# ltiao/bore

Measured on NVIDIA B200. Metric: mlp_value_and_input_grad_evals_per_sec, higher is better.
Workload: dtype f32 MLP / f64 L-BFGS-B

## Files before the change

### bore_b200/csrc/mlp_eval.cu

```cuda
#include <algorithm>

#include <stdlib.h>

#include "common.cuh"
#include "act.cuh"

namespace {

template <int UGB>
struct Map {
  static constexpr int UG = 1 << UGB;
  static constexpr int PG = 32 >> UGB;
  static constexpr int TP = 4 * PG;
  static constexpr int CH = 4 * UG;
  static constexpr int AST = TP + 4;
};

struct SmemPlan {
  int wf[BORE_MAX_LAYERS];
  int bias[BORE_MAX_LAYERS];
  int wl;
  int weights_total;
  int buf[BORE_MAX_LAYERS];
  int warp_total;
  int wl_len;
};

__host__ __device__ inline int rup(int a, int b) { return (a + b - 1) / b * b; }

__host__ __device__ inline void make_plan(const MlpDesc &d, bool grad, int CH, int AST, SmemPlan &p) {
  int off = 0;
  const int G = d.n_layers - 1;
  for (int l = 0; l < G; ++l) {
    int in = d.dims[l], out = d.dims[l + 1];
    p.wf[l] = off; off += (grad ? rup(in, CH) : rup(in, 4)) * (rup(out, CH) + 4);
    p.bias[l] = off; off += rup(out, CH);
  }
  p.wl_len = G > 0 ? rup(d.dims[G], CH) : rup(d.dims[0], CH / 4);
  p.wl = off; off += p.wl_len;
  p.weights_total = rup(off, 4);
  int w = 0;
  p.buf[0] = 0; w += AST * (G > 0 ? rup(d.dims[0], 4) : p.wl_len);
  for (int l = 1; l <= G; ++l) { p.buf[l] = w; w += AST * rup(d.dims[l], CH); }
  p.warp_total = w;
}

__device__ __forceinline__ uint64_t pk2(float lo, float hi) {
  uint64_t r;
  asm("mov.b64 %0, {%1, %2};" : "=l"(r) : "f"(lo), "f"(hi));
  return r;
}
__device__ __forceinline__ void fma2(uint64_t &c, uint64_t a, uint64_t b) {
  asm("fma.rn.f32x2 %0, %1, %2, %0;" : "+l"(c) : "l"(a), "l"(b));
}
__device__ __forceinline__ float2 upk2(uint64_t v) {
  float2 r;
  asm("mov.b64 {%0, %1}, %2;" : "=f"(r.x), "=f"(r.y) : "l"(v));
  return r;
}

template <int AST, bool F2>
__device__ __forceinline__ void tile_gemm(const float *__restrict__ A, const float *__restrict__ W,
                                          int K4, int ldw, float (&acc)[4][4]) {
  if (F2) {
    uint64_t c2[2][4];
#pragma unroll
    for (int u = 0; u < 4; ++u) { c2[0][u] = pk2(acc[0][u], acc[1][u]); c2[1][u] = pk2(acc[2][u], acc[3][u]); }
#pragma unroll 2
    for (int k = 0; k < K4; k += 4) {
      float4 a[4], w[4];
#pragma unroll
      for (int kk = 0; kk < 4; ++kk) {
        a[kk] = *reinterpret_cast<const float4 *>(A + (k + kk) * AST);
        w[kk] = *reinterpret_cast<const float4 *>(W + (k + kk) * ldw);
      }
#pragma unroll
      for (int kk = 0; kk < 4; ++kk) {
        const uint64_t a01 = pk2(a[kk].x, a[kk].y), a23 = pk2(a[kk].z, a[kk].w);
        const float wv[4] = {w[kk].x, w[kk].y, w[kk].z, w[kk].w};
#pragma unroll
        for (int u = 0; u < 4; ++u) {
          const uint64_t ww = pk2(wv[u], wv[u]);
          fma2(c2[0][u], a01, ww);
          fma2(c2[1][u], a23, ww);
        }
      }
    }
#pragma unroll
    for (int u = 0; u < 4; ++u) {
      const float2 lo = upk2(c2[0][u]), hi = upk2(c2[1][u]);
      acc[0][u] = lo.x; acc[1][u] = lo.y; acc[2][u] = hi.x; acc[3][u] = hi.y;
    }
    return;
  }
#pragma unroll 2
  for (int k = 0; k < K4; k += 4) {
    float4 a[4], w[4];
#pragma unroll
    for (int kk = 0; kk < 4; ++kk) {
      a[kk] = *reinterpret_cast<const float4 *>(A + (k + kk) * AST);
      w[kk] = *reinterpret_cast<const float4 *>(W + (k + kk) * ldw);
    }
#pragma unroll
    for (int kk = 0; kk < 4; ++kk) {
      const float av[4] = {a[kk].x, a[kk].y, a[kk].z, a[kk].w};
      const float wv[4] = {w[kk].x, w[kk].y, w[kk].z, w[kk].w};
#pragma unroll
      for (int i = 0; i < 4; ++i)
#pragma unroll
        for (int u = 0; u < 4; ++u) acc[i][u] = fmaf(av[i], wv[u], acc[i][u]);
    }
  }
}

template <int AST, int RS, bool F2>
__device__ __forceinline__ void tile_gemm_T(const float *__restrict__ A, const float *__restrict__ Wrow,
                                            int J4, int ldw, float (&acc)[4][4]) {
  if (F2) {
    uint64_t c2[2][4];
#pragma unroll
    for (int u = 0; u < 4; ++u) { c2[0][u] = pk2(acc[0][u], acc[1][u]); c2[1][u] = pk2(acc[2][u], acc[3][u]); }
#pragma unroll 2
    for (int j = 0; j < J4; j += 4) {
      float4 a[4], w[4];
#pragma unroll
      for (int jj = 0; jj < 4; ++jj) a[jj] = *reinterpret_cast<const float4 *>(A + (j + jj) * AST);
#pragma unroll
      for (int u = 0; u < 4; ++u) w[u] = *reinterpret_cast<const float4 *>(Wrow + u * RS * ldw + j);
#pragma unroll
      for (int jj = 0; jj < 4; ++jj) {
        const uint64_t a01 = pk2(a[jj].x, a[jj].y), a23 = pk2(a[jj].z, a[jj].w);
#pragma unroll
        for (int u = 0; u < 4; ++u) {
          const float wv = jj == 0 ? w[u].x : jj == 1 ? w[u].y : jj == 2 ? w[u].z : w[u].w;
          const uint64_t ww = pk2(wv, wv);
          fma2(c2[0][u], a01, ww);
          fma2(c2[1][u], a23, ww);
        }
      }
    }
#pragma unroll
    for (int u = 0; u < 4; ++u) {
      const float2 lo = upk2(c2[0][u]), hi = upk2(c2[1][u]);
      acc[0][u] = lo.x; acc[1][u] = lo.y; acc[2][u] = hi.x; acc[3][u] = hi.y;
    }
    return;
  }
#pragma unroll 2
  for (int j = 0; j < J4; j += 4) {
    float4 a[4], w[4];
#pragma unroll
    for (int jj = 0; jj < 4; ++jj) a[jj] = *reinterpret_cast<const float4 *>(A + (j + jj) * AST);
#pragma unroll
    for (int u = 0; u < 4; ++u) w[u] = *reinterpret_cast<const float4 *>(Wrow + u * RS * ldw + j);
#pragma unroll
    for (int jj = 0; jj < 4; ++jj) {
      const float av[4] = {a[jj].x, a[jj].y, a[jj].z, a[jj].w};
#pragma unroll
      for (int u = 0; u < 4; ++u) {
        const float wv = jj == 0 ? w[u].x : jj == 1 ? w[u].y : jj == 2 ? w[u].z : w[u].w;
#pragma unroll
        for (int i = 0; i < 4; ++i) acc[i][u] = fmaf(av[i], wv, acc[i][u]);
      }
    }
  }
}

__global__ void __launch_bounds__(256)
mlp_pack_kernel(const MlpDesc d, const SmemPlan P, int CH, int grad, const float *__restrict__ params_all,
                float *__restrict__ packed_all) {
  const float *params = params_all + (size_t)blockIdx.x * d.n_params;
  float *out = packed_all + (size_t)blockIdx.x * P.weights_total;
  const int G = d.n_layers - 1;
  const int tid = threadIdx.x, nthr = blockDim.x;
  for (int l = 0; l < G; ++l) {
    const int in = d.dims[l], outd = d.dims[l + 1];
    const int rows = grad ? rup(in, CH) : rup(in, 4), outP = rup(outd, CH), ld = outP + 4;
    const float *Wg = params + d.w_off[l];
    float *wf = out + P.wf[l];
    for (int e = tid; e < rows * ld; e += nthr) {
      const int k = e / ld, j = e - k * ld;
      wf[e] = (k < in && j < outd) ? Wg[k * outd + j] : 0.f;
    }
    float *bs = out + P.bias[l];
    for (int e = tid; e < outP; e += nthr) bs[e] = e < outd ? params[d.b_off[l] + e] : 0.f;
  }
  {
    const int in = d.dims[G];
    float *wl = out + P.wl;
    for (int e = tid; e < P.weights_total - P.wl; e += nthr)
      wl[e] = e < in ? params[d.w_off[G] + e] : 0.f;
  }
}

__device__ __forceinline__ uint32_t smem_addr(const void *p) { return (uint32_t)__cvta_generic_to_shared(p); }

template <bool GRAD, int UGB, bool F2, bool EXT>
__global__ void __launch_bounds__(512)
mlp_eval_kernel(const MlpDesc d, const SmemPlan P, const float *__restrict__ params,
                const float *__restrict__ packed, const float *__restrict__ X,
                int S, const int *__restrict__ n_dev, const int *__restrict__ list,
                float *__restrict__ f_out, float *__restrict__ g_out, int transform, float sign,
                int per_model, const int *__restrict__ flags) {
  extern __shared__ __align__(128) float smem[];
  __shared__ __align__(8) uint64_t s_bar;
  using M = Map<UGB>;
  constexpr int TP = M::TP, AST = M::AST, CH = M::CH, UG = M::UG;
  const int G = d.n_layers - 1;
  const int tid = threadIdx.x, nthr = blockDim.x;
  const bool multi = per_model > 0;
  int n, tile0, tile_step;
  long row_base = 0;
  int *llist = reinterpret_cast<int *>(smem + P.weights_total + (nthr >> 5) * P.warp_total);
  if (multi) {
    params += (size_t)blockIdx.x * d.n_params;
    packed += (size_t)blockIdx.x * P.weights_total;
    row_base = (long)blockIdx.x * per_model;
    if (flags) {
      __shared__ int s_cnt;
      if (tid == 0) s_cnt = 0;
      __syncthreads();
      for (int c0 = 0; c0 < per_model; c0 += nthr) {
        const int i = c0 + tid;
        const bool on = i < per_model && flags[row_base + i] != 0;
        const unsigned b = __ballot_sync(0xffffffffu, on);
        int wbase = 0;
        if ((tid & 31) == 0 && b) wbase = atomicAdd(&s_cnt, __popc(b));
        wbase = __shfl_sync(0xffffffffu, wbase, 0);
        if (on) llist[wbase + __popc(b & ((1u << (tid & 31)) - 1u))] = i;
      }
      __syncthreads();
      n = s_cnt;
      list = llist;
    } else {
      n = per_model;
      list = nullptr;
    }
    if (n == 0) return;
    tile0 = 0;
    tile_step = nthr >> 5;
  } else {
    n = n_dev ? min(*n_dev, S) : S;
    if (blockIdx.x * (nthr >> 5) * TP >= n) return;
    tile0 = blockIdx.x * (nthr >> 5);
    tile_step = gridDim.x * (nthr >> 5);
  }

  if (tid == 0) {
    const uint32_t bar = smem_addr(&s_bar);
    const uint32_t total = (uint32_t)P.weights_total * sizeof(float);
    asm volatile("mbarrier.init.shared::cta.b64 [%0], 1;" ::"r"(bar) : "memory");
    asm volatile("fence.mbarrier_init.release.cluster;" ::: "memory");
    asm volatile("mbarrier.arrive.expect_tx.shared::cta.b64 _, [%0], %1;" ::"r"(bar), "r"(total) : "memory");
    for (uint32_t off = 0; off < total; off += 65536u) {
      const uint32_t nb = total - off < 65536u ? total - off : 65536u;
      asm volatile("cp.async.bulk.shared::cluster.global.mbarrier::complete_tx::bytes [%0], [%1], %2, [%3];"
                   ::"r"(smem_addr(smem) + off), "l"(reinterpret_cast<const char *>(packed) + off), "r"(nb),
                     "r"(bar)
                   : "memory");
    }
  }
  __syncthreads();
  {
    const uint32_t bar = smem_addr(&s_bar);
    asm volatile(
        "{\n"
        ".reg .pred p;\n"
        "W_WAIT:\n"
        "mbarrier.try_wait.parity.shared::cta.b64 p, [%0], 0;\n"
        "@p bra W_DONE;\n"
        "bra W_WAIT;\n"
        "W_DONE:\n"
        "}\n" ::"r"(bar)
        : "memory");
  }
  const float b_last = params[d.b_off[G]];
  const int act_last = d.act[G];

  const int n_tiles = (n + TP - 1) / TP;
  const int warp = tid >> 5, lane = tid & 31, nwarps = nthr >> 5;
  const int ug = lane & (UG - 1), pg = lane >> UGB;
  float *strip = smem + P.weights_total + warp * P.warp_total;
  const int D = d.dims[0];
  const float *wl = smem + P.wl;

  for (int tile = tile0 + warp; tile < n_tiles; tile += tile_step) {
    const int p0 = tile * TP;
    {
      float *xb = strip + P.buf[0];
      const int rows0 = G > 0 ? rup(D, 4) : P.wl_len;
      for (int pl = 0; pl < TP; ++pl) {
        const int idx = p0 + pl;
        const bool ok = idx < n;
        const long row = ok ? row_base + (list ? list[idx] : idx) : 0;
        for (int k = lane; k < rows0; k += 32)
          xb[k * AST + pl] = (ok && k < D) ? X[row * D + k] : 0.f;
      }
    }
    __syncwarp();

    for (int l = 0; l < G; ++l) {
      const int in4 = rup(d.dims[l], 4), outP = rup(d.dims[l + 1], CH);
      const float *A = strip + P.buf[l] + pg * 4;
      float *H = strip + P.buf[l + 1];
      const float *W = smem + P.wf[l];
      const float *bs = smem + P.bias[l];
      const int a = d.act[l];
      for (int c = 0; c < outP; c += CH) {
        float acc[4][4] = {};
        tile_gemm<AST, F2>(A, W + c + ug * 4, in4, outP + 4, acc);
#pragma unroll
        for (int u = 0; u < 4; ++u) {
          const int unit = c + ug * 4 + u;
          const float b = bs[unit];
          float4 o;
          o.x = act_fwd<EXT>(a, acc[0][u] + b);
          o.y = act_fwd<EXT>(a, acc[1][u] + b);
          o.z = act_fwd<EXT>(a, acc[2][u] + b);
          o.w = act_fwd<EXT>(a, acc[3][u] + b);
          *reinterpret_cast<float4 *>(H + unit * AST + pg * 4) = o;
        }
      }
      __syncwarp();
    }

    float *HL = strip + P.buf[G];
    float up[4] = {0.f, 0.f, 0.f, 0.f};
    for (int k = ug; k < P.wl_len; k += UG) {
      const float4 hv = *reinterpret_cast<const float4 *>(HL + k * AST + pg * 4);
      const float w = wl[k];
      up[0] = fmaf(hv.x, w, up[0]);
      up[1] = fmaf(hv.y, w, up[1]);
      up[2] = fmaf(hv.z, w, up[2]);
      up[3] = fmaf(hv.w, w, up[3]);
    }
#pragma unroll
    for (int i = 0; i < 4; ++i) {
#pragma unroll
      for (int o = 1; o < UG; o <<= 1) up[i] += __shfl_xor_sync(0xffffffffu, up[i], o);
    }
    float dpre[4];
#pragma unroll
    for (int i = 0; i < 4; ++i) {
      const float u = act_fwd<EXT>(act_last, up[i] + b_last);
      float fval, dT;
      if (GRAD) {
        const float v = sign * u;
        if (transform == BORE_TRANSFORM_SIGMOID) {
          fval = 1.f / (1.f + expf(-v));
          dT = fval * (1.f - fval);
        } else if (transform == BORE_TRANSFORM_EXP) {
          fval = expf(v);
          dT = fval;
        } else {
          fval = v;
          dT = 1.f;
        }
        dpre[i] = dT * sign * act_bwd<EXT>(act_last, u);
      } else {
        fval = u;
      }
      const int idx = p0 + pg * 4 + i;
      if (ug == 0 && idx < n) f_out[row_base + (list ? list[idx] : idx)] = fval;
    }
    if (!GRAD) { __syncwarp(); continue; }

    if (G == 0) {
      for (int k = ug; k < D; k += UG) {
        const float w = wl[k];
#pragma unroll
        for (int i = 0; i < 4; ++i) {
          const int idx = p0 + pg * 4 + i;
          if (idx < n) g_out[(row_base + (list ? list[idx] : idx)) * D + k] = dpre[i] * w;
        }
      }
      __syncwarp();
      continue;
    }
    {
      const int a = d.act[G - 1];
      for (int k = ug; k < P.wl_len; k += UG) {
        float4 hv = *reinterpret_cast<const float4 *>(HL + k * AST + pg * 4);
        const float w = wl[k];
        hv.x = dpre[0] * w * act_bwd<EXT>(a, hv.x);
        hv.y = dpre[1] * w * act_bwd<EXT>(a, hv.y);
        hv.z = dpre[2] * w * act_bwd<EXT>(a, hv.z);
        hv.w = dpre[3] * w * act_bwd<EXT>(a, hv.w);
        *reinterpret_cast<float4 *>(HL + k * AST + pg * 4) = hv;
      }
    }
    __syncwarp();
    for (int l = G - 1; l >= 0; --l) {
      const int out4 = rup(d.dims[l + 1], 4), inP = rup(d.dims[l], CH), ldw = rup(d.dims[l + 1], CH) + 4;
      const float *A = strip + P.buf[l + 1] + pg * 4;
      const float *W = smem + P.wf[l];
      float *Hin = strip + P.buf[l];
      if (l > 0) {
        const int a = d.act[l - 1];
        for (int c = 0; c < inP; c += CH) {
          float acc[4][4] = {};
          tile_gemm_T<AST, UG, F2>(A, W + (c + ug) * ldw, out4, ldw, acc);
#pragma unroll
          for (int u = 0; u < 4; ++u) {
            float *hp = Hin + (c + ug + UG * u) * AST + pg * 4;
            float4 hv = *reinterpret_cast<const float4 *>(hp);
            hv.x = acc[0][u] * act_bwd<EXT>(a, hv.x);
            hv.y = acc[1][u] * act_bwd<EXT>(a, hv.y);
            hv.z = acc[2][u] * act_bwd<EXT>(a, hv.z);
            hv.w = acc[3][u] * act_bwd<EXT>(a, hv.w);
            *reinterpret_cast<float4 *>(hp) = hv;
          }
        }
        __syncwarp();
      } else {
        for (int c = 0; c < inP; c += CH) {
          float acc[4][4] = {};
          tile_gemm_T<AST, UG, F2>(A, W + (c + ug) * ldw, out4, ldw, acc);
#pragma unroll
          for (int u = 0; u < 4; ++u) {
            const int k = c + ug + UG * u;
            if (k < rup(D, 4))
              *reinterpret_cast<float4 *>(Hin + k * AST + pg * 4) =
                  make_float4(acc[0][u], acc[1][u], acc[2][u], acc[3][u]);
          }
        }
        __syncwarp();
        for (int pl = 0; pl < TP; ++pl) {
          const int idx = p0 + pl;
          if (idx >= n) break;
          const long row = row_base + (list ? list[idx] : idx);
          for (int k = lane; k < D; k += 32) g_out[row * D + k] = Hin[k * AST + pl];
        }
        __syncwarp();
      }
    }
  }
}

}

static int variant_index(bool grad, int UGB) { return (grad ? 2 : 0) + (UGB == 4 ? 1 : 0); }

template <bool GRAD, int UGB>
static int pack_variant(const bore_mlp *h, int model0, int n_models, cudaStream_t stream) {
  using M = Map<UGB>;
  SmemPlan P;
  make_plan(h->desc, GRAD, M::CH, M::AST, P);
  const int v = variant_index(GRAD, UGB);
  MlpPackCache *pc = h->pack;
  BORE_CHECK(pc != nullptr, "handle has no pack cache");
  const size_t need = (size_t)h->n_models * P.weights_total;
  if (pc->cap[v] < need) {
    if (pc->buf[v]) BORE_CUDA(cudaFree(pc->buf[v]));
    pc->buf[v] = nullptr; pc->cap[v] = 0;
    BORE_CUDA(cudaMalloc(&pc->buf[v], need * sizeof(float)));
    pc->cap[v] = need;
  }
  mlp_pack_kernel<<<n_models, 256, 0, stream>>>(h->desc, P, M::CH, GRAD ? 1 : 0,
                                                 h->params + (size_t)model0 * h->desc.n_params,
                                                 pc->buf[v] + (size_t)model0 * P.weights_total);
  BORE_CUDA(cudaGetLastError());
  return 0;
}

constexpr int EVAL_MAX_SMEM = 227 * 1024;
constexpr int EVAL_STATIC_SMEM = 256;

static size_t eval_smem_bytes(const SmemPlan &P, int warps, size_t list_bytes) {
  return (size_t)(P.weights_total + warps * P.warp_total) * sizeof(float) + list_bytes;
}

template <bool GRAD, int UGB>
static int launch_variant(const bore_mlp *h, const MlpDesc &d, int model0, const float *X,
                          int S, float *f, float *g, const int *list, const int *n_dev,
                          int transform, float sign, int n_models, int per_model, const int *flags,
                          int prepacked, cudaStream_t stream) {
  using M = Map<UGB>;
  SmemPlan P;
  make_plan(d, GRAD, M::CH, M::AST, P);
  const int max_smem = EVAL_MAX_SMEM;
  const bool multi = per_model > 0;
  const size_t list_bytes = (multi && flags) ? (size_t)per_model * sizeof(int) : 0;
  int warps = 16;
  if (multi) warps = std::min(16, std::max(1, (per_model + M::TP - 1) / M::TP));
  while (warps > 1 && eval_smem_bytes(P, warps, list_bytes) + EVAL_STATIC_SMEM > (size_t)max_smem) --warps;
  const size_t smem = eval_smem_bytes(P, warps, list_bytes);
  BORE_CHECK(smem + EVAL_STATIC_SMEM <= (size_t)max_smem, "mlp_eval: model needs %zu B of shared memory (> %d)",
             smem + EVAL_STATIC_SMEM, max_smem);
  if (!prepacked && pack_variant<GRAD, UGB>(h, model0, n_models, stream)) return -1;
  const float *params = h->params + (size_t)model0 * d.n_params;
  const float *packed = h->pack->buf[variant_index(GRAD, UGB)] + (size_t)model0 * P.weights_total;
  int grid;
  if (multi) {
    grid = n_models;
  } else {
    const int n_tiles = (S + M::TP - 1) / M::TP;
    int ctas_needed = (n_tiles + warps - 1) / warps;
    int per_sm = (int)((size_t)max_smem / (smem + 1024));
    if (per_sm < 1) per_sm = 1;
    if (per_sm * warps > 48) per_sm = 48 / warps > 0 ? 48 / warps : 1;
    grid = h->sm_count * per_sm;
    if (grid > ctas_needed) grid = ctas_needed;
    if (grid < 1) grid = 1;
  }
  static const bool f2 = [] { const char *e = getenv("BORE_K2_FFMA2"); return !(e && e[0] == '0'); }();
  const bool ext = acts_ext(d.act, d.n_layers);
  const auto kernel = f2 ? (ext ? mlp_eval_kernel<GRAD, UGB, true, true> : mlp_eval_kernel<GRAD, UGB, true, false>)
                         : (ext ? mlp_eval_kernel<GRAD, UGB, false, true> : mlp_eval_kernel<GRAD, UGB, false, false>);
  static bool attr_done[2][2][64] = {};
  if (h->device >= 64 || !attr_done[f2][ext][h->device]) {
    BORE_CUDA(cudaFuncSetAttribute(kernel, cudaFuncAttributeMaxDynamicSharedMemorySize, max_smem - 256));
    if (h->device < 64) attr_done[f2][ext][h->device] = true;
  }
  kernel<<<grid, warps * 32, smem, stream>>>(d, P, params, packed, X, S, n_dev, list, f, g, transform, sign, per_model,
                                             flags);
  BORE_CUDA(cudaGetLastError());
  return 0;
}

static bool is_wide(const MlpDesc &d) {
  int widest = 0;
  for (int l = 1; l < d.n_layers; ++l) widest = d.dims[l] > widest ? d.dims[l] : widest;
  return widest > 32;
}

static int dispatch(const bore_mlp *h, int model0, bool want_grad, int transform, int negate,
                    const float *X, int S, float *f, float *g, const int *list, const int *n_dev,
                    int n_models, int per_model, const int *flags, int prepacked, cudaStream_t stream) {
  const MlpDesc &d = h->desc;
  const bool wide = is_wide(d);
  const float sign = negate ? -1.f : 1.f;
#define BORE_EVAL(G_, U_)                                                                             \
  launch_variant<G_, U_>(h, d, model0, X, S, f, g, list, n_dev, transform, sign, n_models, per_model, \
                         flags, prepacked, stream)
  if (want_grad) return wide ? BORE_EVAL(true, 4) : BORE_EVAL(true, 3);
  return wide ? BORE_EVAL(false, 4) : BORE_EVAL(false, 3);
#undef BORE_EVAL
}

int mlp_eval_check_envelope(const MlpDesc &d) {
  const bool wide = is_wide(d);
  for (int grad = 0; grad < 2; ++grad) {
    SmemPlan P;
    if (wide) make_plan(d, grad != 0, Map<4>::CH, Map<4>::AST, P);
    else make_plan(d, grad != 0, Map<3>::CH, Map<3>::AST, P);
    const size_t need = eval_smem_bytes(P, 1, 0) + EVAL_STATIC_SMEM;
    BORE_CHECK(need <= (size_t)EVAL_MAX_SMEM,
               "bore_mlp_create: %s needs %zu B of shared memory for one warp (limit %d B)",
               grad ? "value and gradient (K2)" : "predict (K0)", need, EVAL_MAX_SMEM);
  }
  return 0;
}

int mlp_eval_prepare(const bore_mlp *h, int model0, int n_models, bool want_grad, cudaStream_t stream) {
  const bool wide = is_wide(h->desc);
  if (want_grad)
    return wide ? pack_variant<true, 4>(h, model0, n_models, stream)
                : pack_variant<true, 3>(h, model0, n_models, stream);
  return wide ? pack_variant<false, 4>(h, model0, n_models, stream)
              : pack_variant<false, 3>(h, model0, n_models, stream);
}

int launch_mlp_eval(const bore_mlp *h, int model, bool want_grad, int transform, int negate,
                    const float *X, int S, float *f, float *g, const int *list,
                    const int *n_dev, cudaStream_t stream, int prepacked) {
  if (S <= 0) return 0;
  return dispatch(h, model, want_grad, transform, negate, X, S, f, g, list, n_dev, 1, 0, nullptr,
                  prepacked, stream);
}

int launch_mlp_eval_multi(const bore_mlp *h, int model0, int n_models, int per_model, bool want_grad,
                          int transform, int negate, const float *X, float *f, float *g,
                          const int *flags, cudaStream_t stream, int prepacked) {
  if (n_models <= 0 || per_model <= 0) return 0;
  return dispatch(h, model0, want_grad, transform, negate, X, n_models * per_model, f, g, nullptr,
                  nullptr, n_models, per_model, flags, prepacked, stream);
}
```

Before: 46.64 million.

## Prefetch input tiles with cp.async, specialize uniform-width layers, write grads directly

```diff
diff --git a/bore_b200/csrc/mlp_eval.cu b/bore_b200/csrc/mlp_eval.cu
--- a/bore_b200/csrc/mlp_eval.cu
+++ b/bore_b200/csrc/mlp_eval.cu
@@ -59,109 +59,80 @@
   return r;
 }
 
-template <int AST, bool F2>
-__device__ __forceinline__ void tile_gemm(const float *__restrict__ A, const float *__restrict__ W,
-                                          int K4, int ldw, float (&acc)[4][4]) {
-  if (F2) {
+template <bool WT>
+__device__ __forceinline__ float wsel(const float4 (&w)[4], int kk, int u) {
+  const float4 v = WT ? w[u] : w[kk];
+  const int e = WT ? kk : u;
+  return e == 0 ? v.x : e == 1 ? v.y : e == 2 ? v.z : v.w;
+}
+template <bool WT>
+__device__ __forceinline__ void kstep2(uint64_t (&c2)[2][4], const float4 (&a)[4], const float4 (&w)[4]) {
+#pragma unroll
+  for (int kk = 0; kk < 4; ++kk) {
+    const uint64_t a01 = pk2(a[kk].x, a[kk].y), a23 = pk2(a[kk].z, a[kk].w);
+#pragma unroll
+    for (int u = 0; u < 4; ++u) {
+      const float wv = wsel<WT>(w, kk, u);
+      const uint64_t ww = pk2(wv, wv);
+      fma2(c2[0][u], a01, ww);
+      fma2(c2[1][u], a23, ww);
+    }
+  }
+}
+template <bool WT>
+__device__ __forceinline__ void kstep1(float (&acc)[4][4], const float4 (&a)[4], const float4 (&w)[4]) {
+#pragma unroll
+  for (int kk = 0; kk < 4; ++kk) {
+    const float av[4] = {a[kk].x, a[kk].y, a[kk].z, a[kk].w};
+#pragma unroll
+    for (int u = 0; u < 4; ++u) {
+      const float wv = wsel<WT>(w, kk, u);
+#pragma unroll
+      for (int i = 0; i < 4; ++i) acc[i][u] = fmaf(av[i], wv, acc[i][u]);
+    }
+  }
+}
+
+template <int AST, int RS, bool WT, bool F2, int KC, int LDW>
+__device__ __forceinline__ void tile_gemm(const float *__restrict__ A, const float *__restrict__ W, int K4, int ldw,
+                                          float (&acc)[4][4]) {
+  if (KC) K4 = KC;
+  if (LDW) ldw = LDW;
+  constexpr int UNR = KC ? 4 : 2;
+  auto load = [&](int k, float4 (&a)[4], float4 (&w)[4]) {
+#pragma unroll
+    for (int kk = 0; kk < 4; ++kk) a[kk] = *reinterpret_cast<const float4 *>(A + (k + kk) * AST);
+#pragma unroll
+    for (int q = 0; q < 4; ++q)
+      w[q] = *reinterpret_cast<const float4 *>(WT ? W + q * RS * ldw + k : W + (k + q) * ldw);
+  };
+  float4 a[4], w[4];
+  load(0, a, w);
+  if constexpr (F2) {
     uint64_t c2[2][4];
 #pragma unroll
     for (int u = 0; u < 4; ++u) { c2[0][u] = pk2(acc[0][u], acc[1][u]); c2[1][u] = pk2(acc[2][u], acc[3][u]); }
-#pragma unroll 2
+#pragma unroll UNR
     for (int k = 0; k < K4; k += 4) {
-      float4 a[4], w[4];
-#pragma unroll
-      for (int kk = 0; kk < 4; ++kk) {
-        a[kk] = *reinterpret_cast<const float4 *>(A + (k + kk) * AST);
-        w[kk] = *reinterpret_cast<const float4 *>(W + (k + kk) * ldw);
-      }
-#pragma unroll
-      for (int kk = 0; kk < 4; ++kk) {
-        const uint64_t a01 = pk2(a[kk].x, a[kk].y), a23 = pk2(a[kk].z, a[kk].w);
-        const float wv[4] = {w[kk].x, w[kk].y, w[kk].z, w[kk].w};
-#pragma unroll
-        for (int u = 0; u < 4; ++u) {
-          const uint64_t ww = pk2(wv[u], wv[u]);
-          fma2(c2[0][u], a01, ww);
-          fma2(c2[1][u], a23, ww);
-        }
-      }
+      float4 an[4], wn[4];
+      load(k + 4 < K4 ? k + 4 : k, an, wn);
+      kstep2<WT>(c2, a, w);
+#pragma unroll
+      for (int q = 0; q < 4; ++q) { a[q] = an[q]; w[q] = wn[q]; }
     }
 #pragma unroll
     for (int u = 0; u < 4; ++u) {
       const float2 lo = upk2(c2[0][u]), hi = upk2(c2[1][u]);
       acc[0][u] = lo.x; acc[1][u] = lo.y; acc[2][u] = hi.x; acc[3][u] = hi.y;
     }
-    return;
-  }
-#pragma unroll 2
-  for (int k = 0; k < K4; k += 4) {
-    float4 a[4], w[4];
-#pragma unroll
-    for (int kk = 0; kk < 4; ++kk) {
-      a[kk] = *reinterpret_cast<const float4 *>(A + (k + kk) * AST);
-      w[kk] = *reinterpret_cast<const float4 *>(W + (k + kk) * ldw);
-    }
-#pragma unroll
-    for (int kk = 0; kk < 4; ++kk) {
-      const float av[4] = {a[kk].x, a[kk].y, a[kk].z, a[kk].w};
-      const float wv[4] = {w[kk].x, w[kk].y, w[kk].z, w[kk].w};
-#pragma unroll
-      for (int i = 0; i < 4; ++i)
-#pragma unroll
-        for (int u = 0; u < 4; ++u) acc[i][u] = fmaf(av[i], wv[u], acc[i][u]);
-    }
-  }
-}
-
-template <int AST, int RS, bool F2>
-__device__ __forceinline__ void tile_gemm_T(const float *__restrict__ A, const float *__restrict__ Wrow,
-                                            int J4, int ldw, float (&acc)[4][4]) {
-  if (F2) {
-    uint64_t c2[2][4];
-#pragma unroll
-    for (int u = 0; u < 4; ++u) { c2[0][u] = pk2(acc[0][u], acc[1][u]); c2[1][u] = pk2(acc[2][u], acc[3][u]); }
-#pragma unroll 2
-    for (int j = 0; j < J4; j += 4) {
-      float4 a[4], w[4];
-#pragma unroll
-      for (int jj = 0; jj < 4; ++jj) a[jj] = *reinterpret_cast<const float4 *>(A + (j + jj) * AST);
-#pragma unroll
-      for (int u = 0; u < 4; ++u) w[u] = *reinterpret_cast<const float4 *>(Wrow + u * RS * ldw + j);
-#pragma unroll
-      for (int jj = 0; jj < 4; ++jj) {
-        const uint64_t a01 = pk2(a[jj].x, a[jj].y), a23 = pk2(a[jj].z, a[jj].w);
-#pragma unroll
-        for (int u = 0; u < 4; ++u) {
-          const float wv = jj == 0 ? w[u].x : jj == 1 ? w[u].y : jj == 2 ? w[u].z : w[u].w;
-          const uint64_t ww = pk2(wv, wv);
-          fma2(c2[0][u], a01, ww);
-          fma2(c2[1][u], a23, ww);
-        }
-      }
-    }
-#pragma unroll
-    for (int u = 0; u < 4; ++u) {
-      const float2 lo = upk2(c2[0][u]), hi = upk2(c2[1][u]);
-      acc[0][u] = lo.x; acc[1][u] = lo.y; acc[2][u] = hi.x; acc[3][u] = hi.y;
-    }
-    return;
-  }
-#pragma unroll 2
-  for (int j = 0; j < J4; j += 4) {
-    float4 a[4], w[4];
-#pragma unroll
-    for (int jj = 0; jj < 4; ++jj) a[jj] = *reinterpret_cast<const float4 *>(A + (j + jj) * AST);
-#pragma unroll
-    for (int u = 0; u < 4; ++u) w[u] = *reinterpret_cast<const float4 *>(Wrow + u * RS * ldw + j);
-#pragma unroll
-    for (int jj = 0; jj < 4; ++jj) {
-      const float av[4] = {a[jj].x, a[jj].y, a[jj].z, a[jj].w};
-#pragma unroll
-      for (int u = 0; u < 4; ++u) {
-        const float wv = jj == 0 ? w[u].x : jj == 1 ? w[u].y : jj == 2 ? w[u].z : w[u].w;
-#pragma unroll
-        for (int i = 0; i < 4; ++i) acc[i][u] = fmaf(av[i], wv, acc[i][u]);
-      }
+  } else {
+#pragma unroll UNR
+    for (int k = 0; k < K4; k += 4) {
+      float4 an[4], wn[4];
+      load(k + 4 < K4 ? k + 4 : k, an, wn);
+      kstep1<WT>(acc, a, w);
+#pragma unroll
+      for (int q = 0; q < 4; ++q) { a[q] = an[q]; w[q] = wn[q]; }
     }
   }
 }
@@ -195,7 +166,12 @@
 
 __device__ __forceinline__ uint32_t smem_addr(const void *p) { return (uint32_t)__cvta_generic_to_shared(p); }
 
-template <bool GRAD, int UGB, bool F2, bool EXT>
+__device__ __forceinline__ void cp_async4_zfill(float *dst, const float *src, int src_bytes) {
+  asm volatile("cp.async.ca.shared.global [%0], [%1], 4, %2;" ::"r"(smem_addr(dst)), "l"(src), "r"(src_bytes)
+               : "memory");
+}
+
+template <bool GRAD, int UGB, bool F2, bool EXT, int HW>
 __global__ void __launch_bounds__(512)
 mlp_eval_kernel(const MlpDesc d, const SmemPlan P, const float *__restrict__ params,
                 const float *__restrict__ packed, const float *__restrict__ X,
@@ -206,16 +182,17 @@
   __shared__ __align__(8) uint64_t s_bar;
   using M = Map<UGB>;
   constexpr int TP = M::TP, AST = M::AST, CH = M::CH, UG = M::UG;
+  static_assert(HW % CH == 0, "a width class is a whole number of chunks");
   const int G = d.n_layers - 1;
   const int tid = threadIdx.x, nthr = blockDim.x;
   const bool multi = per_model > 0;
   int n, tile0, tile_step;
-  long row_base = 0;
+  int row_base = 0;
   int *llist = reinterpret_cast<int *>(smem + P.weights_total + (nthr >> 5) * P.warp_total);
   if (multi) {
     params += (size_t)blockIdx.x * d.n_params;
     packed += (size_t)blockIdx.x * P.weights_total;
-    row_base = (long)blockIdx.x * per_model;
+    row_base = blockIdx.x * per_model;
     if (flags) {
       __shared__ int s_cnt;
       if (tid == 0) s_cnt = 0;
@@ -245,6 +222,31 @@
     tile0 = blockIdx.x * (nthr >> 5);
     tile_step = gridDim.x * (nthr >> 5);
   }
+
+  const int n_tiles = (n + TP - 1) / TP;
+  const int warp = tid >> 5, lane = tid & 31;
+  const int ug = lane & (UG - 1), pg = lane >> UGB;
+  float *strip = smem + P.weights_total + warp * P.warp_total;
+  const int D = d.dims[0];
+  const int rows0 = G > 0 ? rup(D, 4) : P.wl_len;
+
+  auto tile_row = [&](int tile) {
+    const int idx = tile * TP + lane;
+    return (lane < TP && tile < n_tiles && idx < n) ? row_base + (list ? list[idx] : idx) : -1;
+  };
+  auto gather = [&](int my_row) {
+    float *xb = strip + P.buf[0];
+#pragma unroll 1
+    for (int pl = 0; pl < TP; ++pl) {
+      const int row = __shfl_sync(0xffffffffu, my_row, pl);
+      for (int k = lane; k < rows0; k += 32) {
+        const bool ok = row >= 0 && k < D;
+        cp_async4_zfill(xb + k * AST + pl, ok ? X + (size_t)row * D + k : X, ok ? 4 : 0);
+      }
+    }
+  };
+  int row_next = tile_row(tile0 + warp);
+  if (tile0 + warp < n_tiles) gather(row_next);
 
   if (tid == 0) {
     const uint32_t bar = smem_addr(&s_bar);
@@ -276,39 +278,31 @@
   }
   const float b_last = params[d.b_off[G]];
   const int act_last = d.act[G];
-
-  const int n_tiles = (n + TP - 1) / TP;
-  const int warp = tid >> 5, lane = tid & 31, nwarps = nthr >> 5;
-  const int ug = lane & (UG - 1), pg = lane >> UGB;
-  float *strip = smem + P.weights_total + warp * P.warp_total;
-  const int D = d.dims[0];
   const float *wl = smem + P.wl;
+  constexpr int LS = HW * (HW + 4) + HW;
+  auto wf_of = [&](int l) { return HW ? (l ? P.wf[1] + (l - 1) * LS : P.wf[0]) : P.wf[l]; };
+  auto bias_of = [&](int l) { return HW ? (l ? P.wf[1] + (l - 1) * LS + HW * (HW + 4) : P.bias[0]) : P.bias[l]; };
+  auto buf_of = [&](int l) { return HW ? (l ? P.buf[1] + (l - 1) * AST * HW : P.buf[0]) : P.buf[l]; };
+  const int wl_len = HW && G > 0 ? HW : P.wl_len;
 
   for (int tile = tile0 + warp; tile < n_tiles; tile += tile_step) {
-    const int p0 = tile * TP;
-    {
-      float *xb = strip + P.buf[0];
-      const int rows0 = G > 0 ? rup(D, 4) : P.wl_len;
-      for (int pl = 0; pl < TP; ++pl) {
-        const int idx = p0 + pl;
-        const bool ok = idx < n;
-        const long row = ok ? row_base + (list ? list[idx] : idx) : 0;
-        for (int k = lane; k < rows0; k += 32)
-          xb[k * AST + pl] = (ok && k < D) ? X[row * D + k] : 0.f;
-      }
-    }
+    const int row_cur = row_next;
+    const bool more = tile + tile_step < n_tiles;
+    row_next = tile_row(tile + tile_step);
+    asm volatile("cp.async.wait_all;" ::: "memory");
     __syncwarp();
 
     for (int l = 0; l < G; ++l) {
-      const int in4 = rup(d.dims[l], 4), outP = rup(d.dims[l + 1], CH);
-      const float *A = strip + P.buf[l] + pg * 4;
-      float *H = strip + P.buf[l + 1];
-      const float *W = smem + P.wf[l];
-      const float *bs = smem + P.bias[l];
+      const float *A = strip + buf_of(l) + pg * 4;
+      float *H = strip + buf_of(l + 1);
+      const float *W = smem + wf_of(l);
+      const float *bs = smem + bias_of(l);
       const int a = d.act[l];
+      const int in4 = l ? rup(d.dims[l], 4) : rup(D, 4), outP = HW ? HW : rup(d.dims[l + 1], CH);
       for (int c = 0; c < outP; c += CH) {
         float acc[4][4] = {};
-        tile_gemm<AST, F2>(A, W + c + ug * 4, in4, outP + 4, acc);
+        if (HW && l) tile_gemm<AST, 1, false, F2, HW, HW + 4>(A, W + c + ug * 4, in4, outP + 4, acc);
+        else tile_gemm<AST, 1, false, F2, 0, HW ? HW + 4 : 0>(A, W + c + ug * 4, in4, outP + 4, acc);
 #pragma unroll
         for (int u = 0; u < 4; ++u) {
           const int unit = c + ug * 4 + u;
@@ -322,11 +316,12 @@
         }
       }
       __syncwarp();
-    }
-
-    float *HL = strip + P.buf[G];
+      if (l == 0 && more) gather(row_next);
+    }
+
+    float *HL = strip + buf_of(G);
     float up[4] = {0.f, 0.f, 0.f, 0.f};
-    for (int k = ug; k < P.wl_len; k += UG) {
+    for (int k = ug; k < wl_len; k += UG) {
       const float4 hv = *reinterpret_cast<const float4 *>(HL + k * AST + pg * 4);
       const float w = wl[k];
       up[0] = fmaf(hv.x, w, up[0]);
@@ -339,6 +334,13 @@
 #pragma unroll
       for (int o = 1; o < UG; o <<= 1) up[i] += __shfl_xor_sync(0xffffffffu, up[i], o);
     }
+    if (G == 0) {
+      __syncwarp();
+      if (more) gather(row_next);
+    }
+    int row[4];
+#pragma unroll
+    for (int i = 0; i < 4; ++i) row[i] = __shfl_sync(0xffffffffu, row_cur, pg * 4 + i);
     float dpre[4];
 #pragma unroll
     for (int i = 0; i < 4; ++i) {
@@ -360,8 +362,7 @@
       } else {
         fval = u;
       }
-      const int idx = p0 + pg * 4 + i;
-      if (ug == 0 && idx < n) f_out[row_base + (list ? list[idx] : idx)] = fval;
+      if (ug == 0 && row[i] >= 0) f_out[row[i]] = fval;
     }
     if (!GRAD) { __syncwarp(); continue; }
 
@@ -369,17 +370,15 @@
       for (int k = ug; k < D; k += UG) {
         const float w = wl[k];
 #pragma unroll
-        for (int i = 0; i < 4; ++i) {
-          const int idx = p0 + pg * 4 + i;
-          if (idx < n) g_out[(row_base + (list ? list[idx] : idx)) * D + k] = dpre[i] * w;
-        }
+        for (int i = 0; i < 4; ++i)
+          if (row[i] >= 0) g_out[(size_t)row[i] * D + k] = dpre[i] * w;
       }
       __syncwarp();
       continue;
     }
     {
       const int a = d.act[G - 1];
-      for (int k = ug; k < P.wl_len; k += UG) {
+      for (int k = ug; k < wl_len; k += UG) {
         float4 hv = *reinterpret_cast<const float4 *>(HL + k * AST + pg * 4);
         const float w = wl[k];
         hv.x = dpre[0] * w * act_bwd<EXT>(a, hv.x);
@@ -391,15 +390,16 @@
     }
     __syncwarp();
     for (int l = G - 1; l >= 0; --l) {
-      const int out4 = rup(d.dims[l + 1], 4), inP = rup(d.dims[l], CH), ldw = rup(d.dims[l + 1], CH) + 4;
-      const float *A = strip + P.buf[l + 1] + pg * 4;
-      const float *W = smem + P.wf[l];
-      float *Hin = strip + P.buf[l];
+      const int out4 = HW ? HW : rup(d.dims[l + 1], 4), ldw = (HW ? HW : rup(d.dims[l + 1], CH)) + 4;
+      const int inP = l ? (HW ? HW : rup(d.dims[l], CH)) : rup(D, CH);
+      const float *A = strip + buf_of(l + 1) + pg * 4;
+      const float *W = smem + wf_of(l);
       if (l > 0) {
+        float *Hin = strip + buf_of(l);
         const int a = d.act[l - 1];
         for (int c = 0; c < inP; c += CH) {
           float acc[4][4] = {};
-          tile_gemm_T<AST, UG, F2>(A, W + (c + ug) * ldw, out4, ldw, acc);
+          tile_gemm<AST, UG, true, F2, HW, HW ? HW + 4 : 0>(A, W + (c + ug) * ldw, out4, ldw, acc);
 #pragma unroll
           for (int u = 0; u < 4; ++u) {
             float *hp = Hin + (c + ug + UG * u) * AST + pg * 4;
@@ -415,21 +415,16 @@
       } else {
         for (int c = 0; c < inP; c += CH) {
           float acc[4][4] = {};
-          tile_gemm_T<AST, UG, F2>(A, W + (c + ug) * ldw, out4, ldw, acc);
+          tile_gemm<AST, UG, true, F2, HW, HW ? HW + 4 : 0>(A, W + (c + ug) * ldw, out4, ldw, acc);
 #pragma unroll
           for (int u = 0; u < 4; ++u) {
             const int k = c + ug + UG * u;
-            if (k < rup(D, 4))
-              *reinterpret_cast<float4 *>(Hin + k * AST + pg * 4) =
-                  make_float4(acc[0][u], acc[1][u], acc[2][u], acc[3][u]);
+            if (k < D) {
+#pragma unroll
+              for (int i = 0; i < 4; ++i)
+                if (row[i] >= 0) g_out[(size_t)row[i] * D + k] = acc[i][u];
+            }
           }
-        }
-        __syncwarp();
-        for (int pl = 0; pl < TP; ++pl) {
-          const int idx = p0 + pl;
-          if (idx >= n) break;
-          const long row = row_base + (list ? list[idx] : idx);
-          for (int k = lane; k < D; k += 32) g_out[row * D + k] = Hin[k * AST + pl];
         }
         __syncwarp();
       }
@@ -468,6 +463,19 @@
 
 static size_t eval_smem_bytes(const SmemPlan &P, int warps, size_t list_bytes) {
   return (size_t)(P.weights_total + warps * P.warp_total) * sizeof(float) + list_bytes;
+}
+
+static int width_class(const MlpDesc &d) {
+  const int w = d.n_layers > 1 ? d.dims[1] : 0;
+  for (int l = 2; l < d.n_layers; ++l)
+    if (d.dims[l] != w) return 0;
+  return (w == 32 || w == 64 || w == 128) ? w : 0;
+}
+
+template <bool GRAD, int UGB, int HW>
+static auto kernel_for(bool f2, bool ext) {
+  return f2 ? (ext ? mlp_eval_kernel<GRAD, UGB, true, true, HW> : mlp_eval_kernel<GRAD, UGB, true, false, HW>)
+            : (ext ? mlp_eval_kernel<GRAD, UGB, false, true, HW> : mlp_eval_kernel<GRAD, UGB, false, false, HW>);
 }
 
 template <bool GRAD, int UGB>
@@ -505,12 +513,16 @@
   }
   static const bool f2 = [] { const char *e = getenv("BORE_K2_FFMA2"); return !(e && e[0] == '0'); }();
   const bool ext = acts_ext(d.act, d.n_layers);
-  const auto kernel = f2 ? (ext ? mlp_eval_kernel<GRAD, UGB, true, true> : mlp_eval_kernel<GRAD, UGB, true, false>)
-                         : (ext ? mlp_eval_kernel<GRAD, UGB, false, true> : mlp_eval_kernel<GRAD, UGB, false, false>);
-  static bool attr_done[2][2][64] = {};
-  if (h->device >= 64 || !attr_done[f2][ext][h->device]) {
+  constexpr int C1 = M::CH, C2 = UGB == 4 ? 2 * M::CH : 0;
+  const int hw = width_class(d);
+  const int cls = hw == C1 ? 1 : (C2 && hw == C2) ? 2 : 0;
+  const auto kernel = cls == 1   ? kernel_for<GRAD, UGB, C1>(f2, ext)
+                      : cls == 2 ? kernel_for<GRAD, UGB, C2>(f2, ext)
+                                 : kernel_for<GRAD, UGB, 0>(f2, ext);
+  static bool attr_done[3][2][2][64] = {};
+  if (h->device >= 64 || !attr_done[cls][f2][ext][h->device]) {
     BORE_CUDA(cudaFuncSetAttribute(kernel, cudaFuncAttributeMaxDynamicSharedMemorySize, max_smem - 256));
-    if (h->device < 64) attr_done[f2][ext][h->device] = true;
+    if (h->device < 64) attr_done[cls][f2][ext][h->device] = true;
   }
   kernel<<<grid, warps * 32, smem, stream>>>(d, P, params, packed, X, S, n_dev, list, f, g, transform, sign, per_model,
                                              flags);
```

Result: faster. 47.89 million, median of 6 (+2.7%).
